# ChaissonLab/LRA

Hardware: AMD Instinct MI355X
Metric: aligned Gbp/s, 30 kb ONT vs GRCh38 (MapRead_lowacc end to end incl. SAM text), per job (higher is better)
Workload: dtype int32

## Files before the change

### lra_amd/csrc/sdp.hip

```cpp
#include "common.h"
#include <type_traits>
#include "scan.h"
#include <algorithm>
#include <cmath>
#include <cstring>
#include <cstdlib>
#include <string>
#include <vector>
#include <rocprim/rocprim.hpp>

namespace {

constexpr int LV = 18;
constexpr uint32_t NONE = 0xFFFFFFFFu;
constexpr int MAXALN = 16;

__device__ __forceinline__ void wave_sync() {
  __builtin_amdgcn_fence(__ATOMIC_RELEASE, "workgroup");
  __builtin_amdgcn_wave_barrier();
  __builtin_amdgcn_fence(__ATOMIC_ACQUIRE, "workgroup");
}
__device__ __forceinline__ int wave_incl_scan(int v, int lane) {
  (void)lane;
#define LRA_DPP_ADD(ctrl_, rmask_) v += __builtin_amdgcn_update_dpp(0, v, (ctrl_), (rmask_), 0xf, false)
  LRA_DPP_ADD(0x111, 0xf);
  LRA_DPP_ADD(0x112, 0xf);
  LRA_DPP_ADD(0x114, 0xf);
// ... 196 lines not shown
  const float rt = rate_in ? rate_in[r] : rate;
  for (uint64_t g = fragOff[r] + threadIdx.x; g < fragOff[r + 1]; g += blockDim.x) { fval[g] = flen[g] * rt; fprevNode[g] = NONE; fprevInd[g] = NONE; fflags[g] = 3; }
  if (threadIdx.x == 0) status[r] = 0;
}

struct BuildArgs {
  int r0, n;
  const uint32_t* order;
  const uint64_t* ptOff;
  const uint32_t* hq; const uint32_t* ht; const uint8_t* hfl; const uint32_t* h2; const uint64_t* key3; const uint32_t* pay3;
  uint32_t* scratch;
  uint32_t* cntEntries; uint32_t* cntNodes; uint32_t* cntD; uint32_t* cntV; uint32_t* cntRC;
  const ReadArena* ra;
  uint32_t* status;
  unsigned long long* stat;
};

template <int NW>
__device__ __forceinline__ int blk_incl_scan(int v, int lane, int wave, int* s_w, int& total) {
  const int inc = wave_incl_scan(v, lane);
  if (NW == 1) { total = __builtin_amdgcn_readlane(inc, 63); return inc; }
  if (lane == 63) s_w[wave] = inc;
  __syncthreads();
  int pre = 0, tot = 0;
#pragma unroll
  for (int w = 0; w < NW; w++) { const int x = s_w[w]; tot += x; if (w < wave) pre += x; }
  __syncthreads();
  total = tot;
  return inc + pre;
}
template <bool EMIT, int NW, int MODE = 0, int OCC = 8, bool BSTAT = false>
__global__ void __launch_bounds__(64 * NW, NW == 1 ? OCC : 1) sdp_build(BuildArgs a) {
  constexpr int NT = 64 * NW;
  constexpr bool LDSV = MODE == 1, NARROW = MODE != 0;
  using IT = typename std::conditional<NARROW, uint16_t, uint32_t>::type;
  using DT = typename std::conditional<NARROW, uint32_t, long long>::type;
  constexpr IT INONE = (IT)~(IT)0;
  extern __shared__ __attribute__((aligned(16))) char dyn_lds[];
  __shared__ int s_w[4][NW == 1 ? 1 : NW];
  __shared__ unsigned long long s_bt[BSTAT ? 8 : 1];
  unsigned long long btPrev = 0;
  constexpr bool bstat = BSTAT;
  if (bstat) { if (threadIdx.x < 8) s_bt[threadIdx.x] = 0; btPrev = __builtin_amdgcn_s_memtime(); }
#define BTICK(k_) do { if (bstat) { const unsigned long long t__ = __builtin_amdgcn_s_memtime(); if (threadIdx.x == 0) s_bt[k_] += t__ - btPrev; btPrev = t__; } } while (0)
  const int rr = (int)a.order[blockIdx.x], r = a.r0 + rr, tid = threadIdx.x, lane = tid & 63, wave = tid >> 6;
  auto SYNC = [&]() { if (NW == 1) wave_sync(); else __syncthreads(); };
  const uint64_t p0 = a.ptOff[r], pc0 = a.ptOff[a.r0];
  const int P = (int)(a.ptOff[r + 1] - p0);
  if (P == 0) { if (tid == 0) { if (!EMIT) { a.cntEntries[rr] = 0; a.cntNodes[rr] = 0; a.cntD[rr] = 0; } a.cntV[rr] = 0; a.cntRC[rr] = 0; } return; }
  const uint32_t* hq = a.hq + p0; const uint32_t* ht = a.ht + p0; const uint32_t* h2 = a.h2 + p0;
  const uint64_t* key3 = a.key3 + p0; const uint32_t* pay3 = a.pay3 + p0;
  uint32_t* S = a.scratch + 34 * (p0 - pc0) + 64 * (uint64_t)rr;
  const int NCAP = P + 2;
  uint32_t* tbl = S + 8 * P + 2;
  uint32_t* tmp = tbl + 12 * NCAP;
  IT* eb_ = LDSV ? (IT*)dyn_lds : (IT*)S;
  IT* rowOf = eb_; IT* colOf = rowOf + P;
  IT* lp = colOf + P;
  IT* ln = lp + 2 * P;
  IT* pf = ln + 2 * P;
  IT* ph = pf + P + 1;
  IT* ll = NARROW ? ph + P + 1 : (IT*)(tmp + 8 * NCAP);
  DT* ld = LDSV ? (DT*)(dyn_lds + ((((size_t)(10 * P + 2) * sizeof(IT)) + 7) & ~(size_t)7)) : NARROW ? (DT*)(tmp + 8 * NCAP) : (DT*)(ll + 2 * P);
  auto LN = [&](int idx) -> uint32_t { const IT v = ln[idx]; return v == INONE ? NONE : (uint32_t)v; };
#define TB(c, f, k) tbl[((c) * 6 + (f)) * NCAP + (k)]
#define TM(f, k) tmp[(f) * NCAP + (k)]
  enum { F_LS, F_LE, F_SB, F_SE, F_EB, F_EE };
  enum { T_C1S, T_C1E, T_ND, T_NE, T_CH0, T_CH1, T_BASE, T_GID };
  int R = 0, C = 0;
  for (int i0 = 0; i0 < P; i0 += NT) {
    const int i = i0 + tid;
    const int head = (i < P) && (i == 0 || hq[i] != hq[i - 1]);
    int tot; const int inc = blk_incl_scan<NW>(head, lane, wave, s_w[0], tot);
    if (i < P) rowOf[i] = R + inc - 1;
    R += tot;
  }
  for (int i0 = 0; i0 < P; i0 += NT) {
    const int i = i0 + tid;
    const int head = (i < P) && (i == 0 || ht[h2[i]] != ht[h2[i - 1]]);
    int tot; const int inc = blk_incl_scan<NW>(head, lane, wave, s_w[0], tot);
    if (i < P) colOf[h2[i]] = C + inc - 1;
// ... 32 lines not shown
    const bool col = fam & 1, back = fam >= 2, desc = (fam == 1 || fam == 2), swapped = (fam == 3);
    const IT* lineOf = col ? colOf : rowOf;
    const int nLines = col ? C : R;
    const int sc = back ? 2 : 0;
    const int nS = cOff[sc + 1] - cOff[sc], nEn = cOff[sc + 2] - cOff[sc + 1], Pf = nS + nEn;
    if (nS == 0 || nEn == 0) continue;
    const int fam2 = fam & 1;
    const int dSide = swapped ? 1 : 0, eSide = swapped ? 0 : 1;
    for (int i = tid; i < Pf; i += NT) {
      const uint32_t pos = pay3[cOff[sc] + i];
      lp[i] = (IT)pos; ln[i] = 0; ll[i] = lineOf[pos];
      ld[i] = (DT)(back ? (long long)ht[pos] + hq[pos] : (long long)ht[pos] - hq[pos]);
    }
    if (tid == 0) { TB(0, F_LS, 0) = 0; TB(0, F_LE, 0) = nLines; TB(0, F_SB, 0) = 0; TB(0, F_SE, 0) = nS; TB(0, F_EB, 0) = nS; TB(0, F_EE, 0) = Pf; }
    int nNodes = 1, cur = 0;
    SYNC();
    BTICK(7);
    for (int level = 0; nNodes > 0 && !outgrown; level++) {
      if (level >= LV) { overflow = true; break; }
      const int nxt = cur ^ 1;
      IT* lpc = lp + cur * P; IT* lpn = lp + nxt * P;
      IT* llc = ll + cur * P; IT* lln = ll + nxt * P;
      DT* ldc = ld + (size_t)cur * P; DT* ldn = ld + (size_t)nxt * P;
      {
        int carry = 0;
        constexpr int UA = 4;
        for (int i0 = 0; i0 < Pf; i0 += UA * NT) {
          uint32_t kk[UA]; uint32_t ss[UA], ee[UA]; IT lv[UA]; int ff[UA];
#pragma unroll
          for (int u = 0; u < UA; u++) { const int i = i0 + u * NT + tid; kk[u] = i < Pf ? LN(i) : NONE; lv[u] = i < Pf ? llc[i] : (IT)0; }
#pragma unroll
          for (int u = 0; u < UA; u++) { ss[u] = 0; ee[u] = 0; if (kk[u] != NONE) { ss[u] = TB(cur, F_LS, kk[u]); ee[u] = TB(cur, F_LE, kk[u]); } }
#pragma unroll
          for (int u = 0; u < UA; u++) ff[u] = kk[u] == NONE ? 0 : (ee[u] - ss[u] > 1) ? (lv[u] < ((ss[u] + ee[u]) >> 1)) : 1;
#pragma unroll
          for (int u = 0; u < UA; u++) {
            const int i = i0 + u * NT + tid;
            if (i0 + u * NT >= Pf) break;
            int tot; const int inc = blk_incl_scan<NW>(ff[u], lane, wave, s_w[0], tot);
            if (i < Pf) pf[i] = (IT)(carry + inc - ff[u]);
            carry += tot;
          }
        }
        if (tid == 0) pf[Pf] = (IT)carry;
      }
      SYNC();
      BTICK(1);
      for (int k = tid; k < nNodes; k += NT) {
        TM(T_C1S, k) = (uint32_t)pf[TB(cur, F_SE, k)] - (uint32_t)pf[TB(cur, F_SB, k)];
        TM(T_C1E, k) = (uint32_t)pf[TB(cur, F_EE, k)] - (uint32_t)pf[TB(cur, F_EB, k)];
      }
      SYNC();
      {
        constexpr int UC = 2;
        for (int i0 = 0; i0 < Pf; i0 += UC * NT) {
          uint32_t kk[UC], pi0[UC], pi1[UC], sb[UC], c1[UC], psb[UC]; IT vlp[UC], vll[UC]; DT vld[UC];
#pragma unroll
          for (int u = 0; u < UC; u++) {
            const int i = i0 + u * NT + tid;
            kk[u] = NONE; pi0[u] = 0; pi1[u] = 0; vlp[u] = 0; vll[u] = 0; vld[u] = 0;
            if (i < Pf) { kk[u] = LN(i); pi0[u] = (uint32_t)pf[i]; pi1[u] = (uint32_t)pf[i + 1]; vlp[u] = lpc[i]; vll[u] = llc[i]; vld[u] = ldc[i]; }
          }
#pragma unroll
          for (int u = 0; u < UC; u++) {
            const int i = i0 + u * NT + tid;
            const bool isS = i < nS;
            sb[u] = 0; c1[u] = 0;
            if (kk[u] != NONE) { sb[u] = isS ? TB(cur, F_SB, kk[u]) : TB(cur, F_EB, kk[u]); c1[u] = isS ? TM(T_C1S, kk[u]) : TM(T_C1E, kk[u]); }
          }
#pragma unroll
          for (int u = 0; u < UC; u++) psb[u] = kk[u] != NONE ? (uint32_t)pf[sb[u]] : 0;
#pragma unroll
          for (int u = 0; u < UC; u++) {
            const int i = i0 + u * NT + tid;
            if (i >= Pf) continue;
            if (kk[u] == NONE) { ln[P + i] = INONE; continue; }
            const uint32_t rank1 = pi0[u] - psb[u];
            const uint32_t first = pi1[u] - pi0[u];
            const uint32_t np_ = first ? sb[u] + rank1 : sb[u] + c1[u] + ((uint32_t)i - sb[u] - rank1);
            lpn[np_] = vlp[u]; lln[np_] = vll[u]; ldn[np_] = vld[u];
            ln[P + np_] = (IT)(2 * kk[u] + (first ? 0 : 1));
          }
        }
      }
      SYNC();
      BTICK(2);
      {
        int carry = 0;
        constexpr int UD = NW == 1 ? 4 : 2;
        for (int j0 = 0; j0 < Pf; j0 += UD * NT) {
          uint32_t k2v[UD], le[UD], ls[UD], bg[UD], c1[UD]; DT d0[UD], d1[UD]; int hd[UD];
#pragma unroll
          for (int u = 0; u < UD; u++) {
            const int j = j0 + u * NT + tid;
            k2v[u] = NONE; d0[u] = 0; d1[u] = 0;
            if (j < Pf) { k2v[u] = LN(P + j); d0[u] = ldn[j]; d1[u] = j > 0 ? ldn[j - 1] : ldn[j]; }
          }
#pragma unroll
          for (int u = 0; u < UD; u++) {
            const int j = j0 + u * NT + tid;
            const bool isS = j < nS;
            le[u] = 0; ls[u] = 0; bg[u] = 0; c1[u] = 0;
            if (k2v[u] != NONE) {
              const uint32_t k = k2v[u] >> 1;
              le[u] = TB(cur, F_LE, k); ls[u] = TB(cur, F_LS, k); bg[u] = isS ? TB(cur, F_SB, k) : TB(cur, F_EB, k); c1[u] = isS ? TM(T_C1S, k) : TM(T_C1E, k);
            }
          }
#pragma unroll
          for (int u = 0; u < UD; u++) {
            const int j = j0 + u * NT + tid;
            hd[u] = 0;
            if (k2v[u] != NONE) {
              const uint32_t side = k2v[u] & 1;
              const bool isS = j < nS;
              const bool leaf = le[u] - ls[u] == 1;
              const bool in = leaf || (int)side == (isS ? eSide : dSide);
              if (in) {
                uint32_t beg = bg[u];
                if (!leaf && side == 1) beg += c1[u];
                hd[u] = ((uint32_t)j == beg) ? 1 : (d0[u] != d1[u]);
// ... 1 lines not shown
            }
          }
#pragma unroll
          for (int u = 0; u < UD; u++) {
            const int j = j0 + u * NT + tid;
            if (j0 + u * NT >= Pf) break;
            int tot; const int inc = blk_incl_scan<NW>(hd[u], lane, wave, s_w[0], tot);
            if (j < Pf) ph[j] = (IT)(carry + inc - hd[u]);
            carry += tot;
          }
        }
        if (tid == 0) ph[Pf] = (IT)carry;
      }
      SYNC();
      BTICK(3);
      int nNext = 0;
      for (int k0 = 0; k0 < nNodes; k0 += NT) {
        const int k = k0 + tid;
        uint32_t nD = 0, nE = 0, act0 = 0, act1 = 0, full = 0;
        uint32_t ls = 0, le = 0, sb = 0, se = 0, eb = 0, ee = 0, c1S = 0, c1E = 0;
        bool leaf = false;
        if (k < nNodes) {
          ls = TB(cur, F_LS, k); le = TB(cur, F_LE, k); sb = TB(cur, F_SB, k); se = TB(cur, F_SE, k); eb = TB(cur, F_EB, k); ee = TB(cur, F_EE, k);
          c1S = TM(T_C1S, k); c1E = TM(T_C1E, k);
          leaf = le - ls == 1;
          uint32_t dB, dE, eB, eE;
          if (leaf) { dB = eb; dE = ee; eB = sb; eE = se; }
          else {
            dB = dSide == 0 ? eb : eb + c1E; dE = dSide == 0 ? eb + c1E : ee;
            eB = eSide == 0 ? sb : sb + c1S; eE = eSide == 0 ? sb + c1S : se;
          }
          nD = (uint32_t)ph[dE] - (uint32_t)ph[dB]; nE = (uint32_t)ph[eE] - (uint32_t)ph[eB];
          full = nD > 0 && nE > 0;
          if (!leaf) {
            const bool goD = nD > 0, goE = nE > 0;
            if (dSide == 0) { act0 = goD; act1 = goE; } else { act1 = goD; act0 = goE; }
          }
        }
        int totF, totEnt, totD, totC;
        const int incF = blk_incl_scan<NW>((int)full, lane, wave, s_w[0], totF), incEnt = blk_incl_scan<NW>((int)(full ? nD + nE : 0), lane, wave, s_w[1], totEnt),
                  incD = blk_incl_scan<NW>((int)(full ? nD : 0), lane, wave, s_w[2], totD), incC = blk_incl_scan<NW>((int)(act0 + act1), lane, wave, s_w[3], totC);
        if (EMIT && ((uint64_t)nNodesTot + totF > capN || (uint64_t)nEntries + totEnt > capE || (uint64_t)sumD + totD > capD)) { outgrown = true; break; }
        if (k < nNodes) {
          const uint32_t gid = nNodesTot + incF - full, base = nEntries + incEnt - (full ? nD + nE : 0), dpre = sumD + incD - (full ? nD : 0);
          TM(T_ND, k) = nD; TM(T_NE, k) = nE; TM(T_GID, k) = full ? gid : NONE; TM(T_BASE, k) = base;
          uint32_t ci = nNext + incC - (act0 + act1);
          const uint32_t med = (ls + le) >> 1;
          TM(T_CH0, k) = NONE; TM(T_CH1, k) = NONE;
          if (act0) { TM(T_CH0, k) = ci; TB(nxt, F_LS, ci) = ls; TB(nxt, F_LE, ci) = med; TB(nxt, F_SB, ci) = sb; TB(nxt, F_SE, ci) = sb + c1S;
                      TB(nxt, F_EB, ci) = eb; TB(nxt, F_EE, ci) = eb + c1E; ci++; }
          if (act1) { TM(T_CH1, k) = ci; TB(nxt, F_LS, ci) = med; TB(nxt, F_LE, ci) = le; TB(nxt, F_SB, ci) = sb + c1S; TB(nxt, F_SE, ci) = se;
                      TB(nxt, F_EB, ci) = eb + c1E; TB(nxt, F_EE, ci) = ee; }
          if (EMIT && full) {
            Node nd;
            nd.dBase = base; nd.nD = nD; nd.nE = nE; nd.last = -1; nd.sTop = 1; nd.nBlk = 0;
            nd.stkOff = 2 * dpre + 4 * gid; nd.blkOff = blkPair + 2 * base + 8 * gid; nd.stkCap = 2 * nD + 4; nd.blkCap = 2 * (nD + nE) + 8;
            nd.eLast = 0;
            nodesR[gid] = nd;
            stkR[nd.stkOff] = make_int2(-1, (int)nE + 1);
          }
        }
        nNodesTot += totF; nEntries += totEnt; sumD += totD; nNext += totC;
      }
      if (outgrown) break;
      SYNC();
      BTICK(4);
      {
        constexpr int UF = 2;
        for (int j0 = 0; j0 < Pf; j0 += UF * NT) {
          uint32_t k2v[UF], le[UF], ls[UF], ch[UF], gidv[UF], bg[UF], c1[UF], nNE[UF], nND[UF], bs[UF], p0v[UF], p1v[UF], pbg[UF], posv[UF], tq[UF], tt[UF];
#pragma unroll
          for (int u = 0; u < UF; u++) {
            const int j = j0 + u * NT + tid;
            k2v[u] = NONE; p0v[u] = 0; p1v[u] = 0; posv[u] = 0;
            if (j < Pf) { k2v[u] = LN(P + j); if (EMIT) { p0v[u] = (uint32_t)ph[j]; p1v[u] = (uint32_t)ph[j + 1]; posv[u] = lpn[j]; } }
          }
#pragma unroll
          for (int u = 0; u < UF; u++) {
            const int j = j0 + u * NT + tid;
            const bool isS = j < nS;
            le[u] = 0; ls[u] = 0; ch[u] = 0; gidv[u] = NONE; bg[u] = 0; c1[u] = 0; nNE[u] = 0; nND[u] = 0; bs[u] = 0; tq[u] = 0; tt[u] = 0;
            if (k2v[u] != NONE) {
              const uint32_t k = k2v[u] >> 1, side = k2v[u] & 1;
              le[u] = TB(cur, F_LE, k); ls[u] = TB(cur, F_LS, k); ch[u] = side == 0 ? TM(T_CH0, k) : TM(T_CH1, k); gidv[u] = TM(T_GID, k);
              if (EMIT) {
                bg[u] = isS ? TB(cur, F_SB, k) : TB(cur, F_EB, k); c1[u] = isS ? TM(T_C1S, k) : TM(T_C1E, k);
                nNE[u] = TM(T_NE, k); nND[u] = TM(T_ND, k); bs[u] = TM(T_BASE, k);
                tq[u] = hq[posv[u]]; tt[u] = ht[posv[u]];
              }
            }
          }
#pragma unroll
          for (int u = 0; u < UF; u++) {
            pbg[u] = 0;
            if (EMIT && k2v[u] != NONE) {
              const uint32_t side = k2v[u] & 1;
              const bool leaf = le[u] - ls[u] == 1;
              uint32_t beg = bg[u];
              if (!leaf && side == 1) beg += c1[u];
              bg[u] = beg;
              pbg[u] = (uint32_t)ph[beg];
// ... 21 lines not shown
                const uint32_t pos = posv[u];
                if (head) {
                  const long long dgv = back ? (long long)tt[u] + tq[u] : (long long)tt[u] - tq[u];
                  entR[ent].val = dgv;
                  if (isS && idx == n - 1) nodesR[gid].eLast = dgv;
                }
                visR[(uint64_t)pos * (2 * LV) + fam2 * LV + level] = make_uint2(gid, idx);
              }
            }
          }
        }
      }
      SYNC();
      BTICK(5);
      if (EMIT) {
        constexpr int UG = 2;
        for (int j0 = 0; j0 < Pf; j0 += UG * NT) {
          uint32_t k2v[UG], gidv[UG], le[UG], ls[UG], bg[UG], c1[UG], nDv[UG], nEv[UG], bs[UG], p0v[UG], p1v[UG], pbg[UG];
          bool on[UG];
#pragma unroll
          for (int u = 0; u < UG; u++) {
            const int j = j0 + u * NT + tid;
            k2v[u] = NONE; p0v[u] = 0; p1v[u] = 0;
            if (j < Pf) { k2v[u] = LN(P + j); p0v[u] = (uint32_t)ph[j]; p1v[u] = (uint32_t)ph[j + 1]; }
          }
#pragma unroll
          for (int u = 0; u < UG; u++) {
            const int j = j0 + u * NT + tid;
            const bool isS = j < nS;
            gidv[u] = NONE; le[u] = 0; ls[u] = 0; bg[u] = 0; c1[u] = 0; nDv[u] = 0; nEv[u] = 0; bs[u] = 0;
            if (k2v[u] != NONE && p1v[u] != p0v[u]) {
              const uint32_t k = k2v[u] >> 1;
              gidv[u] = TM(T_GID, k); le[u] = TB(cur, F_LE, k); ls[u] = TB(cur, F_LS, k);
              bg[u] = isS ? TB(cur, F_SB, k) : TB(cur, F_EB, k); c1[u] = isS ? TM(T_C1S, k) : TM(T_C1E, k);
              nDv[u] = TM(T_ND, k); nEv[u] = TM(T_NE, k); bs[u] = TM(T_BASE, k);
            }
          }
#pragma unroll
          for (int u = 0; u < UG; u++) {
            const int j = j0 + u * NT + tid;
            const bool isS = j < nS;
            const uint32_t side = k2v[u] & 1;
            const bool leaf = le[u] - ls[u] == 1;
            on[u] = k2v[u] != NONE && p1v[u] != p0v[u] && gidv[u] != NONE && (leaf || (int)side == (isS ? eSide : dSide));
            pbg[u] = 0;
            if (on[u]) { uint32_t beg = bg[u]; if (!leaf && side == 1) beg += c1[u]; pbg[u] = (uint32_t)ph[beg]; }
          }
          uint32_t entv[UG], mv[UG], lo[UG], cnt[UG]; long long xv[UG]; const Ent* opp[UG];
#pragma unroll
// ... 36 lines not shown
                if (cnt[u] > 0) { const uint32_t s2 = cnt[u] >> 1; if (go(vL[u])) { lo[u] += s2 + 1; cnt[u] -= s2 + 1; } else cnt[u] = s2; }
              }
            }
          }
#pragma unroll
          for (int u = 0; u < UG; u++) {
            if (!on[u]) continue;
            const bool isS = j0 + u * NT + tid < nS;
            const uint32_t ent = entv[u], m = mv[u];
            entR[ent].b = isS ? (int32_t)lo[u] - 1 : (lo[u] == m ? -1 : (int32_t)lo[u]);
            if (!isS) edR[ent] = lo[u] == m ? 0 : opp[u][lo[u]].val;
            entR[ent].v = 0.f; apR[ent] = 0;
          }
        }
      }
      nNodes = nNext; cur = nxt;
      SYNC();
      BTICK(6);
    }
  }
  if (bstat && tid == 0) { for (int k = 0; k < 8; k++) atomicAdd(a.stat + k, s_bt[k]); atomicAdd(a.stat + 8, (unsigned long long)P); }
  for (int o = 32; o > 0; o >>= 1) nVisits += __shfl_xor(nVisits, o);
  if (NW > 1) {
    if (lane == 0) s_w[0][wave] = (int)nVisits;
    __syncthreads();
    nVisits = 0;
    for (int w = 0; w < NW; w++) nVisits += (uint32_t)s_w[0][w];
  }
  if (tid == 0) {
    if (!EMIT) { a.cntEntries[rr] = nEntries; a.cntNodes[rr] = nNodesTot; a.cntD[rr] = sumD; a.cntV[rr] = nVisits; a.cntRC[rr] = (uint32_t)max(R, C); }
    else { a.cntV[rr] = nEntries; a.cntRC[rr] = (uint32_t)max(R, C); }
    if (overflow) atomicOr(&a.status[r], (uint32_t)LRA_ST_RANGE);
    if (outgrown) atomicOr(&a.status[r], (uint32_t)LRA_ST_CAPACITY);
  }
#undef TB
#undef TM
#undef BTICK
}

struct ProcArgs {
  int r0, n;
  const uint32_t* order;
  const uint64_t* ptOff; const uint64_t* fragOff;
  const uint8_t* hfl; const uint32_t* hfr;
  const int32_t* flen; float* fval; uint32_t* fprevNode; uint32_t* fprevInd; uint8_t* fflags;
  const float* rate_in; float rate;
  const ReadArena* ra; uint32_t* poolUsed;
  uint32_t* status;
  PwlTab pwl;
  const short* penTab; int penN;
// ... 1056 lines not shown
    a.cq[k] = a.fq[f0 + lf]; a.ct[k] = a.ft[f0 + lf]; a.clen[k] = a.flen[f0 + lf]; a.cstrand[k] = a.fstrand[f0 + lf];
    a.can[k] = a.fai[f0 + lf]; a.ccl[k] = a.fcl[f0 + lf];
  }
  a.nChains[r] = (uint32_t)nCh;
}

inline size_t sz(size_t n, size_t elem) { return (n * elem + 255) / 256 * 256; }

static long sdp_big_points(const lra_ctx* ctx, int mode) {
  if (const char* e = getenv("LRA_SDP_BIG_POINTS")) return atol(e);
  if (ctx->sdp_inner) return 1500;
  if (mode == 0) { if (const char* e = getenv("LRA_SDP_BIG_POINTS_A")) return atol(e); return 2500; }
  if (const char* e = getenv("LRA_SDP_BIG_POINTS_2")) return atol(e);
  return ctx->pipelined ? 14000 : 6000;
}
template <bool EMIT>
static void launch_small_builds(lra_ctx* ctx, const BuildArgs& ba, const uint32_t* d_order, const std::vector<uint32_t>& h_order, const uint64_t* h_pt, int from, int to) {
  static const bool noLds = getenv("LRA_SDP_BUILD_NOLDS") != nullptr;
  hipStream_t st = ctx->stream;
  auto pts = [&](int i) { return (long)(h_pt[h_order[i] + 1] - h_pt[h_order[i]]); };
  int at = from;
  const long caps[3] = {512, 256, 128};
  int cut[4];
  for (int c = 0; c < 3; c++) { while (at < to && (noLds || pts(at) > caps[c])) at++; cut[c] = at; }
  cut[3] = to;
  if (cut[0] > from) {
    int mid = from;
    while (mid < cut[0] && pts(mid) >= 16384) mid++;
    if (mid > from) { BuildArgs bb = ba; bb.order = d_order + from; hipLaunchKernelGGL((sdp_build<EMIT, 1, 0>), dim3(mid - from), dim3(64), 0, st, bb); }
    if (cut[0] > mid) {
      BuildArgs bb = ba; bb.order = d_order + mid;
      static const int occEnv = getenv("LRA_SDP_BUILD_OCC") ? atoi(getenv("LRA_SDP_BUILD_OCC")) : 0;
      const int occ = occEnv ? occEnv : ctx->pipelined ? 6 : 8;
      if (bb.stat) { if (occ == 6) hipLaunchKernelGGL((sdp_build<EMIT, 1, 2, 6, true>), dim3(cut[0] - mid), dim3(64), 0, st, bb); else hipLaunchKernelGGL((sdp_build<EMIT, 1, 2, 8, true>), dim3(cut[0] - mid), dim3(64), 0, st, bb); }
      else if (occ == 4) hipLaunchKernelGGL((sdp_build<EMIT, 1, 2, 4>), dim3(cut[0] - mid), dim3(64), 0, st, bb);
      else if (occ == 5) hipLaunchKernelGGL((sdp_build<EMIT, 1, 2, 5>), dim3(cut[0] - mid), dim3(64), 0, st, bb);
      else if (occ == 6) hipLaunchKernelGGL((sdp_build<EMIT, 1, 2, 6>), dim3(cut[0] - mid), dim3(64), 0, st, bb);
      else hipLaunchKernelGGL((sdp_build<EMIT, 1, 2>), dim3(cut[0] - mid), dim3(64), 0, st, bb);
    }
  }
  for (int c = 0; c < 3; c++) {
    const int n = cut[c + 1] - cut[c];
    if (n <= 0) continue;
    BuildArgs bb = ba; bb.order = d_order + cut[c];
    hipLaunchKernelGGL((sdp_build<EMIT, 1, 1>), dim3(n), dim3(64), (size_t)(28 * caps[c] + 32), st, bb);
  }
}

int sdp_run(lra_ctx* ctx, int n_reads, const uint64_t* d_cluster_off, const uint64_t* d_c_start, const uint32_t* d_c_count,
            const int32_t* d_c_strand, const uint32_t* d_q, const uint32_t* d_t, const int32_t* d_len, const uint64_t* d_read_off,
            const float* d_rate, const lra_sdp_opts* opts, lra_chain_result* out, const uint32_t* d_qe, const uint32_t* d_te,
            const int32_t* d_num_anchors) {
  const bool boxes = d_qe != nullptr;
// ... 184 lines not shown
        for (int i = 0; i < nr; i++) h_order[i] = (uint32_t)i;
        std::sort(h_order.begin(), h_order.end(), [&](uint32_t x, uint32_t y) {
          const uint64_t px = h_pt[r0 + x + 1] - h_pt[r0 + x], py = h_pt[r0 + y + 1] - h_pt[r0 + y];
          return px != py ? px > py : x < y;
        });
      }
      LRA_HIP_CHECK(ctx, hipMemcpyAsync(order, h_order.data(), (size_t)nr * 4, hipMemcpyHostToDevice, st));
      LRA_HIP_CHECK(ctx, hipStreamSynchronize(st));
      h_orderAll = h_order;
    }
    uint64_t* entOff = (uint64_t*)take(ws, nr1 + 1, 8); uint64_t* bytes = (uint64_t*)take(ws, nr1 + 1, 8); uint64_t* byteOff = (uint64_t*)take(ws, nr1 + 1, 8);
    ReadArena* ra = (ReadArena*)take(ws, nr1, sizeof(ReadArena));
    BuildArgs ba;
    memset(&ba, 0, sizeof ba);
    ba.r0 = r0; ba.n = nr; ba.ptOff = ptOff; ba.hq = hq; ba.ht = ht; ba.hfl = hfl; ba.h2 = pay2; ba.key3 = key1; ba.pay3 = pay1; ba.scratch = scratch;
    ba.cntEntries = cntE; ba.cntNodes = cntN; ba.cntD = cntD; ba.cntV = cntV; ba.cntRC = cntRC; ba.status = status; ba.order = order; ba.stat = nullptr;
    static const bool buildStat = getenv("LRA_SDP_BUILD_STAT") != nullptr;
    if (buildStat) { (void)hipMalloc((void**)&ba.stat, 16 * 8); (void)hipMemsetAsync(ba.stat, 0, 16 * 8, st); }
    const bool onePassEnv = !(getenv("LRA_SDP_ONEPASS") && getenv("LRA_SDP_ONEPASS")[0] == '0');
    const bool onePass = onePassEnv && !getenv("LRA_SDP_RATIOS");
    auto count_pass = [&](const uint32_t* d_ord, const std::vector<uint32_t>& h_ord, int n) {
      lra_time_begin(ctx, ctx->sdp_inner ? "sdp_inner_build_count" : "sdp_build_count");
      const long big_pts = sdp_big_points(ctx, opts->mode);
      int nb0 = 0;
      while (nb0 < n && (long)(h_pt[r0 + h_ord[nb0] + 1] - h_pt[r0 + h_ord[nb0]]) >= big_pts) nb0++;
      const bool forked = nb0 > 0 && n > nb0;
      BuildArgs bc = ba; bc.order = d_ord; bc.n = n;
      if (nb0 > 0) hipLaunchKernelGGL((sdp_build<false, 16>), dim3(nb0), dim3(1024), 0, forked ? lra_side_fork(ctx) : st, bc);
      if (n > nb0) launch_small_builds<false>(ctx, bc, d_ord, h_ord, h_pt.data() + r0, nb0, n);
      if (forked) lra_side_join(ctx);
      lra_time_end(ctx);
// ... 164 lines not shown
      h_sub.clear();
      for (int i = 0; i < nsub; i++) { const uint32_t rr = att == 0 ? h_orderAll[i] : h_prev[i]; if (h_status[rr] & LRA_ST_CAPACITY) h_sub.push_back(rr); }
      nsub = (int)h_sub.size();
      if (nsub == 0) break;
      h_prev = h_sub;
      LRA_HIP_CHECK(ctx, hipMemcpyAsync(order2, h_sub.data(), (size_t)nsub * 4, hipMemcpyHostToDevice, st));
      LRA_HIP_CHECK(ctx, hipStreamSynchronize(st));
      subOrder = order2;
    }
    if (ba.stat) {
      unsigned long long hb[16];
      (void)hipStreamSynchronize(st); (void)hipMemcpy(hb, ba.stat, sizeof hb, hipMemcpyDeviceToHost); (void)hipFree(ba.stat); ba.stat = nullptr;
      const double pts = (double)std::max<unsigned long long>(hb[8], 1);
      fprintf(stderr, "[sdp-build-stat] mode %d inner %d reads %d; the wave-per-read builds of 513 .. 16383 points, %llu points; cycles per point: set-up %.1f family %.1f | per level pass A %.1f C %.1f D %.1f E %.1f F %.1f G %.1f\n", opts->mode, (int)ctx->sdp_inner, nr,
              hb[8], hb[0] / pts, hb[7] / pts, hb[1] / pts, hb[2] / pts, hb[3] / pts, hb[4] / pts, hb[5] / pts, hb[6] / pts);
    }
    if (onePass) { int rc = read_rc(); if (rc) return rc; }
    totalEntries += totE;
    const uint64_t cf0 = h_frag[r0], cfn = h_frag[r1] - h_frag[r0];
    if (cfn > 0) {
      lra_time_begin(ctx, ctx->sdp_inner ? "sdp_inner_trace" : "sdp_trace");
      const bool needOrder = opts->mode != LRA_SDP_SINGLE_CLUSTER;
      if (needOrder) hipLaunchKernelGGL(k_valkeys, dim3((unsigned)((cfn + 255) / 256)), dim3(256), 0, st, cf0, cfn, fval, fragRead, fragOff, okey, opay);
      hipLaunchKernelGGL(k_pred, dim3((unsigned)((cfn + 255) / 256)), dim3(256), 0, st, cf0, cfn, r0, (const uint32_t*)fragRead, (const uint32_t*)fprevNode,
                         (const uint32_t*)fprevInd, (const uint32_t*)status, (const ReadArena*)ra, spare);
      lra_time_end(ctx);
      if (needOrder) { int rc = lra_sort_minimizers_batch(ctx, nr, fragOff + r0, okey, opay); if (rc) return rc; }
      TraceArgs ta;
      ta.r0 = r0; ta.n = nr; ta.numAln = opts->NumAln; ta.single = opts->mode == LRA_SDP_SINGLE_CLUSTER; ta.alnthres = opts->alnthres; ta.fragOff = fragOff; ta.read_off = d_read_off; ta.fq = fq; ta.ft = ft;
      ta.flen = flen; ta.fcl = fcl; ta.fai = fai; ta.fval = fval; ta.fpred = spare; ta.fflags = fflags; ta.opay = opay; ta.used = used;
// ... 36 lines not shown
```

Measured before the change: 1.199.

## Finish small SDP build subtrees in LDS once children fit a local cap

The level loop of the sparse DP build kernel becomes a lambda. In MODE 2 it now tracks the largest child node size. Once every child holds at most 62 points, the remaining levels run group by group in LDS: nodes are packed into groups of up to 62 points, their element arrays and node tables are copied from the global arena into LDS, and all deeper levels finish there with unroll factor 1. This aims to cut global-memory traffic for the deep levels of mid-sized reads. In exchange it adds dynamic LDS per block, which may lower occupancy, plus group partitioning and copy overhead; an env var can turn it off.

```diff
diff --git a/lra_amd/csrc/sdp.hip b/lra_amd/csrc/sdp.hip
--- a/lra_amd/csrc/sdp.hip
+++ b/lra_amd/csrc/sdp.hip
@@ -11,6 +11,7 @@
 
 namespace {
 
+constexpr int SUB_CAP = 62;
 constexpr int LV = 18;
 constexpr uint32_t NONE = 0xFFFFFFFFu;
 constexpr int MAXALN = 16;
@@ -237,6 +238,7 @@
   const ReadArena* ra;
   uint32_t* status;
   unsigned long long* stat;
+  int subCap;
 };
 
 template <int NW>
@@ -262,9 +264,10 @@
   extern __shared__ __attribute__((aligned(16))) char dyn_lds[];
   __shared__ int s_w[4][NW == 1 ? 1 : NW];
   __shared__ unsigned long long s_bt[BSTAT ? 8 : 1];
+  __shared__ unsigned long long s_bx[BSTAT ? 5 : 1];
   unsigned long long btPrev = 0;
   constexpr bool bstat = BSTAT;
-  if (bstat) { if (threadIdx.x < 8) s_bt[threadIdx.x] = 0; btPrev = __builtin_amdgcn_s_memtime(); }
+  if (bstat) { if (threadIdx.x < 8) s_bt[threadIdx.x] = 0; if (threadIdx.x < 5) s_bx[threadIdx.x] = 0; btPrev = __builtin_amdgcn_s_memtime(); }
 #define BTICK(k_) do { if (bstat) { const unsigned long long t__ = __builtin_amdgcn_s_memtime(); if (threadIdx.x == 0) s_bt[k_] += t__ - btPrev; btPrev = t__; } } while (0)
   const int rr = (int)a.order[blockIdx.x], r = a.r0 + rr, tid = threadIdx.x, lane = tid & 63, wave = tid >> 6;
   auto SYNC = [&]() { if (NW == 1) wave_sync(); else __syncthreads(); };
@@ -285,9 +288,10 @@
   IT* ph = pf + P + 1;
   IT* ll = NARROW ? ph + P + 1 : (IT*)(tmp + 8 * NCAP);
   DT* ld = LDSV ? (DT*)(dyn_lds + ((((size_t)(10 * P + 2) * sizeof(IT)) + 7) & ~(size_t)7)) : NARROW ? (DT*)(tmp + 8 * NCAP) : (DT*)(ll + 2 * P);
-  auto LN = [&](int idx) -> uint32_t { const IT v = ln[idx]; return v == INONE ? NONE : (uint32_t)v; };
 #define TB(c, f, k) tbl[((c) * 6 + (f)) * NCAP + (k)]
-#define TM(f, k) tmp[(f) * NCAP + (k)]
+#define TBC(f, k) tbC[(f) * NC + (k)]
+#define TBN(f, k) tbN[(f) * NC + (k)]
+#define TM(f, k) tm[(f) * NC + (k)]
   enum { F_LS, F_LE, F_SB, F_SE, F_EB, F_EE };
   enum { T_C1S, T_C1E, T_ND, T_NE, T_CH0, T_CH1, T_BASE, T_GID };
   int R = 0, C = 0;
@@ -350,23 +354,22 @@
     }
     if (tid == 0) { TB(0, F_LS, 0) = 0; TB(0, F_LE, 0) = nLines; TB(0, F_SB, 0) = 0; TB(0, F_SE, 0) = nS; TB(0, F_EB, 0) = nS; TB(0, F_EE, 0) = Pf; }
     int nNodes = 1, cur = 0;
+    int maxCh = Pf;
     SYNC();
     BTICK(7);
-    for (int level = 0; nNodes > 0 && !outgrown; level++) {
-      if (level >= LV) { overflow = true; break; }
-      const int nxt = cur ^ 1;
-      IT* lpc = lp + cur * P; IT* lpn = lp + nxt * P;
-      IT* llc = ll + cur * P; IT* lln = ll + nxt * P;
-      DT* ldc = ld + (size_t)cur * P; DT* ldn = ld + (size_t)nxt * P;
+    auto runLevel = [&](auto inLds, const int level, const int Pf, const int nS, const int PS, auto* lpc, auto* lpn, auto* llc, auto* lln, auto* ldc, auto* ldn,
+                        auto* ln, auto* pf, auto* ph, uint32_t* tbC, uint32_t* tbN, uint32_t* tm, const int NC, const int nNodes, int& maxCh) -> int {
+      constexpr bool L = decltype(inLds)::value;
+      auto LN = [&](int idx) -> uint32_t { const IT v = ln[idx]; return v == INONE ? NONE : (uint32_t)v; };
       {
         int carry = 0;
-        constexpr int UA = 4;
+        constexpr int UA = L ? 1 : 4;
         for (int i0 = 0; i0 < Pf; i0 += UA * NT) {
           uint32_t kk[UA]; uint32_t ss[UA], ee[UA]; IT lv[UA]; int ff[UA];
 #pragma unroll
           for (int u = 0; u < UA; u++) { const int i = i0 + u * NT + tid; kk[u] = i < Pf ? LN(i) : NONE; lv[u] = i < Pf ? llc[i] : (IT)0; }
 #pragma unroll
-          for (int u = 0; u < UA; u++) { ss[u] = 0; ee[u] = 0; if (kk[u] != NONE) { ss[u] = TB(cur, F_LS, kk[u]); ee[u] = TB(cur, F_LE, kk[u]); } }
+          for (int u = 0; u < UA; u++) { ss[u] = 0; ee[u] = 0; if (kk[u] != NONE) { ss[u] = TBC(F_LS, kk[u]); ee[u] = TBC(F_LE, kk[u]); } }
 #pragma unroll
           for (int u = 0; u < UA; u++) ff[u] = kk[u] == NONE ? 0 : (ee[u] - ss[u] > 1) ? (lv[u] < ((ss[u] + ee[u]) >> 1)) : 1;
 #pragma unroll
@@ -383,12 +386,12 @@
       SYNC();
       BTICK(1);
       for (int k = tid; k < nNodes; k += NT) {
-        TM(T_C1S, k) = (uint32_t)pf[TB(cur, F_SE, k)] - (uint32_t)pf[TB(cur, F_SB, k)];
-        TM(T_C1E, k) = (uint32_t)pf[TB(cur, F_EE, k)] - (uint32_t)pf[TB(cur, F_EB, k)];
+        TM(T_C1S, k) = (uint32_t)pf[TBC(F_SE, k)] - (uint32_t)pf[TBC(F_SB, k)];
+        TM(T_C1E, k) = (uint32_t)pf[TBC(F_EE, k)] - (uint32_t)pf[TBC(F_EB, k)];
       }
       SYNC();
       {
-        constexpr int UC = 2;
+        constexpr int UC = L ? 1 : 2;
         for (int i0 = 0; i0 < Pf; i0 += UC * NT) {
           uint32_t kk[UC], pi0[UC], pi1[UC], sb[UC], c1[UC], psb[UC]; IT vlp[UC], vll[UC]; DT vld[UC];
 #pragma unroll
@@ -402,7 +405,7 @@
             const int i = i0 + u * NT + tid;
             const bool isS = i < nS;
             sb[u] = 0; c1[u] = 0;
-            if (kk[u] != NONE) { sb[u] = isS ? TB(cur, F_SB, kk[u]) : TB(cur, F_EB, kk[u]); c1[u] = isS ? TM(T_C1S, kk[u]) : TM(T_C1E, kk[u]); }
+            if (kk[u] != NONE) { sb[u] = isS ? TBC(F_SB, kk[u]) : TBC(F_EB, kk[u]); c1[u] = isS ? TM(T_C1S, kk[u]) : TM(T_C1E, kk[u]); }
           }
 #pragma unroll
           for (int u = 0; u < UC; u++) psb[u] = kk[u] != NONE ? (uint32_t)pf[sb[u]] : 0;
@@ -410,12 +413,12 @@
           for (int u = 0; u < UC; u++) {
             const int i = i0 + u * NT + tid;
             if (i >= Pf) continue;
-            if (kk[u] == NONE) { ln[P + i] = INONE; continue; }
+            if (kk[u] == NONE) { ln[PS + i] = INONE; continue; }
             const uint32_t rank1 = pi0[u] - psb[u];
             const uint32_t first = pi1[u] - pi0[u];
             const uint32_t np_ = first ? sb[u] + rank1 : sb[u] + c1[u] + ((uint32_t)i - sb[u] - rank1);
             lpn[np_] = vlp[u]; lln[np_] = vll[u]; ldn[np_] = vld[u];
-            ln[P + np_] = (IT)(2 * kk[u] + (first ? 0 : 1));
+            ln[PS + np_] = (IT)(2 * kk[u] + (first ? 0 : 1));
           }
         }
       }
@@ -423,14 +426,14 @@
       BTICK(2);
       {
         int carry = 0;
-        constexpr int UD = NW == 1 ? 4 : 2;
+        constexpr int UD = L ? 1 : NW == 1 ? 4 : 2;
         for (int j0 = 0; j0 < Pf; j0 += UD * NT) {
           uint32_t k2v[UD], le[UD], ls[UD], bg[UD], c1[UD]; DT d0[UD], d1[UD]; int hd[UD];
 #pragma unroll
           for (int u = 0; u < UD; u++) {
             const int j = j0 + u * NT + tid;
             k2v[u] = NONE; d0[u] = 0; d1[u] = 0;
-            if (j < Pf) { k2v[u] = LN(P + j); d0[u] = ldn[j]; d1[u] = j > 0 ? ldn[j - 1] : ldn[j]; }
+            if (j < Pf) { k2v[u] = LN(PS + j); d0[u] = ldn[j]; d1[u] = j > 0 ? ldn[j - 1] : ldn[j]; }
           }
 #pragma unroll
           for (int u = 0; u < UD; u++) {
@@ -439,7 +442,7 @@
             le[u] = 0; ls[u] = 0; bg[u] = 0; c1[u] = 0;
             if (k2v[u] != NONE) {
               const uint32_t k = k2v[u] >> 1;
-              le[u] = TB(cur, F_LE, k); ls[u] = TB(cur, F_LS, k); bg[u] = isS ? TB(cur, F_SB, k) : TB(cur, F_EB, k); c1[u] = isS ? TM(T_C1S, k) : TM(T_C1E, k);
+              le[u] = TBC(F_LE, k); ls[u] = TBC(F_LS, k); bg[u] = isS ? TBC(F_SB, k) : TBC(F_EB, k); c1[u] = isS ? TM(T_C1S, k) : TM(T_C1E, k);
             }
           }
 #pragma unroll
@@ -471,14 +474,14 @@
       }
       SYNC();
       BTICK(3);
-      int nNext = 0;
+      int nNext = 0, mc = 0;
       for (int k0 = 0; k0 < nNodes; k0 += NT) {
         const int k = k0 + tid;
         uint32_t nD = 0, nE = 0, act0 = 0, act1 = 0, full = 0;
         uint32_t ls = 0, le = 0, sb = 0, se = 0, eb = 0, ee = 0, c1S = 0, c1E = 0;
         bool leaf = false;
         if (k < nNodes) {
-          ls = TB(cur, F_LS, k); le = TB(cur, F_LE, k); sb = TB(cur, F_SB, k); se = TB(cur, F_SE, k); eb = TB(cur, F_EB, k); ee = TB(cur, F_EE, k);
+          ls = TBC(F_LS, k); le = TBC(F_LE, k); sb = TBC(F_SB, k); se = TBC(F_SE, k); eb = TBC(F_EB, k); ee = TBC(F_EE, k);
           c1S = TM(T_C1S, k); c1E = TM(T_C1E, k);
           leaf = le - ls == 1;
           uint32_t dB, dE, eB, eE;
@@ -504,10 +507,11 @@
           uint32_t ci = nNext + incC - (act0 + act1);
           const uint32_t med = (ls + le) >> 1;
           TM(T_CH0, k) = NONE; TM(T_CH1, k) = NONE;
-          if (act0) { TM(T_CH0, k) = ci; TB(nxt, F_LS, ci) = ls; TB(nxt, F_LE, ci) = med; TB(nxt, F_SB, ci) = sb; TB(nxt, F_SE, ci) = sb + c1S;
-                      TB(nxt, F_EB, ci) = eb; TB(nxt, F_EE, ci) = eb + c1E; ci++; }
-          if (act1) { TM(T_CH1, k) = ci; TB(nxt, F_LS, ci) = med; TB(nxt, F_LE, ci) = le; TB(nxt, F_SB, ci) = sb + c1S; TB(nxt, F_SE, ci) = se;
-                      TB(nxt, F_EB, ci) = eb + c1E; TB(nxt, F_EE, ci) = ee; }
+          if (act0) { TM(T_CH0, k) = ci; TBN(F_LS, ci) = ls; TBN(F_LE, ci) = med; TBN(F_SB, ci) = sb; TBN(F_SE, ci) = sb + c1S;
+                      TBN(F_EB, ci) = eb; TBN(F_EE, ci) = eb + c1E; ci++; }
+          if (act1) { TM(T_CH1, k) = ci; TBN(F_LS, ci) = med; TBN(F_LE, ci) = le; TBN(F_SB, ci) = sb + c1S; TBN(F_SE, ci) = se;
+                      TBN(F_EB, ci) = eb + c1E; TBN(F_EE, ci) = ee; }
+          if (MODE == 2) { if (act0) mc = max(mc, (int)(c1S + c1E)); if (act1) mc = max(mc, (int)(se - sb - c1S + ee - eb - c1E)); }
           if (EMIT && full) {
             Node nd;
             nd.dBase = base; nd.nD = nD; nd.nE = nE; nd.last = -1; nd.sTop = 1; nd.nBlk = 0;
@@ -519,18 +523,19 @@
         }
         nNodesTot += totF; nEntries += totEnt; sumD += totD; nNext += totC;
       }
-      if (outgrown) break;
+      if (outgrown) return 0;
+      if (MODE == 2) { for (int o = 32; o > 0; o >>= 1) mc = max(mc, __shfl_xor(mc, o)); maxCh = __builtin_amdgcn_readfirstlane(mc); }
       SYNC();
       BTICK(4);
       {
-        constexpr int UF = 2;
+        constexpr int UF = L ? 1 : 2;
         for (int j0 = 0; j0 < Pf; j0 += UF * NT) {
           uint32_t k2v[UF], le[UF], ls[UF], ch[UF], gidv[UF], bg[UF], c1[UF], nNE[UF], nND[UF], bs[UF], p0v[UF], p1v[UF], pbg[UF], posv[UF], tq[UF], tt[UF];
 #pragma unroll
           for (int u = 0; u < UF; u++) {
             const int j = j0 + u * NT + tid;
             k2v[u] = NONE; p0v[u] = 0; p1v[u] = 0; posv[u] = 0;
-            if (j < Pf) { k2v[u] = LN(P + j); if (EMIT) { p0v[u] = (uint32_t)ph[j]; p1v[u] = (uint32_t)ph[j + 1]; posv[u] = lpn[j]; } }
+            if (j < Pf) { k2v[u] = LN(PS + j); if (EMIT) { p0v[u] = (uint32_t)ph[j]; p1v[u] = (uint32_t)ph[j + 1]; posv[u] = lpn[j]; } }
           }
 #pragma unroll
           for (int u = 0; u < UF; u++) {
@@ -539,9 +544,9 @@
             le[u] = 0; ls[u] = 0; ch[u] = 0; gidv[u] = NONE; bg[u] = 0; c1[u] = 0; nNE[u] = 0; nND[u] = 0; bs[u] = 0; tq[u] = 0; tt[u] = 0;
             if (k2v[u] != NONE) {
               const uint32_t k = k2v[u] >> 1, side = k2v[u] & 1;
-              le[u] = TB(cur, F_LE, k); ls[u] = TB(cur, F_LS, k); ch[u] = side == 0 ? TM(T_CH0, k) : TM(T_CH1, k); gidv[u] = TM(T_GID, k);
+              le[u] = TBC(F_LE, k); ls[u] = TBC(F_LS, k); ch[u] = side == 0 ? TM(T_CH0, k) : TM(T_CH1, k); gidv[u] = TM(T_GID, k);
               if (EMIT) {
-                bg[u] = isS ? TB(cur, F_SB, k) : TB(cur, F_EB, k); c1[u] = isS ? TM(T_C1S, k) : TM(T_C1E, k);
+                bg[u] = isS ? TBC(F_SB, k) : TBC(F_EB, k); c1[u] = isS ? TM(T_C1S, k) : TM(T_C1E, k);
                 nNE[u] = TM(T_NE, k); nND[u] = TM(T_ND, k); bs[u] = TM(T_BASE, k);
                 tq[u] = hq[posv[u]]; tt[u] = ht[posv[u]];
               }
@@ -593,7 +598,7 @@
       SYNC();
       BTICK(5);
       if (EMIT) {
-        constexpr int UG = 2;
+        constexpr int UG = L ? 1 : 2;
         for (int j0 = 0; j0 < Pf; j0 += UG * NT) {
           uint32_t k2v[UG], gidv[UG], le[UG], ls[UG], bg[UG], c1[UG], nDv[UG], nEv[UG], bs[UG], p0v[UG], p1v[UG], pbg[UG];
           bool on[UG];
@@ -601,7 +606,7 @@
           for (int u = 0; u < UG; u++) {
             const int j = j0 + u * NT + tid;
             k2v[u] = NONE; p0v[u] = 0; p1v[u] = 0;
-            if (j < Pf) { k2v[u] = LN(P + j); p0v[u] = (uint32_t)ph[j]; p1v[u] = (uint32_t)ph[j + 1]; }
+            if (j < Pf) { k2v[u] = LN(PS + j); p0v[u] = (uint32_t)ph[j]; p1v[u] = (uint32_t)ph[j + 1]; }
           }
 #pragma unroll
           for (int u = 0; u < UG; u++) {
@@ -610,8 +615,8 @@
             gidv[u] = NONE; le[u] = 0; ls[u] = 0; bg[u] = 0; c1[u] = 0; nDv[u] = 0; nEv[u] = 0; bs[u] = 0;
             if (k2v[u] != NONE && p1v[u] != p0v[u]) {
               const uint32_t k = k2v[u] >> 1;
-              gidv[u] = TM(T_GID, k); le[u] = TB(cur, F_LE, k); ls[u] = TB(cur, F_LS, k);
-              bg[u] = isS ? TB(cur, F_SB, k) : TB(cur, F_EB, k); c1[u] = isS ? TM(T_C1S, k) : TM(T_C1E, k);
+              gidv[u] = TM(T_GID, k); le[u] = TBC(F_LE, k); ls[u] = TBC(F_LS, k);
+              bg[u] = isS ? TBC(F_SB, k) : TBC(F_EB, k); c1[u] = isS ? TM(T_C1S, k) : TM(T_C1E, k);
               nDv[u] = TM(T_ND, k); nEv[u] = TM(T_NE, k); bs[u] = TM(T_BASE, k);
             }
           }
@@ -678,12 +683,69 @@
           }
         }
       }
-      nNodes = nNext; cur = nxt;
       SYNC();
       BTICK(6);
-    }
-  }
-  if (bstat && tid == 0) { for (int k = 0; k < 8; k++) atomicAdd(a.stat + k, s_bt[k]); atomicAdd(a.stat + 8, (unsigned long long)P); }
+      return nNext;
+    };
+    for (int level = 0; nNodes > 0 && !outgrown; level++) {
+      if (level >= LV) { overflow = true; break; }
+      if constexpr (MODE == 2) {
+        if (a.subCap > 0 && maxCh <= SUB_CAP) {
+          constexpr int CS = SUB_CAP, NC2 = CS;
+          IT* lpL = (IT*)dyn_lds; IT* llL = lpL + 2 * CS; IT* lnL = llL + 2 * CS; IT* pfL = lnL + 2 * CS; IT* phL = pfL + CS + 1;
+          DT* ldL = (DT*)(dyn_lds + (((size_t)(8 * CS + 2) * sizeof(IT) + 7) & ~(size_t)7));
+          const uint32_t* tbL = tbl + cur * 6 * NCAP;
+          uint32_t* tA = (uint32_t*)(ldL + 2 * CS); uint32_t* tB = tA + 6 * NC2; uint32_t* tmL = tB + 6 * NC2;
+          if (bstat && tid == 0) { s_bx[2]++; s_bx[3] += (unsigned long long)level; }
+          int maxLv = level;
+          for (int k0 = 0; k0 < nNodes && !outgrown && !overflow;) {
+            const uint32_t s0 = tbL[F_SB * NCAP + k0], e0 = tbL[F_EB * NCAP + k0];
+            int k1 = nNodes;
+            for (int kb = k0 + 1; kb < nNodes; kb += 64) {
+              const int k = kb + lane;
+              const bool brk = k >= nNodes || (tbL[F_SE * NCAP + k] - s0) + (tbL[F_EE * NCAP + k] - e0) > (uint32_t)CS;
+              const unsigned long long m = __ballot(brk);
+              if (m) { k1 = kb + (int)__builtin_ctzll(m); break; }
+            }
+            k1 = __builtin_amdgcn_readfirstlane(k1);
+            const uint32_t s1 = tbL[F_SE * NCAP + k1 - 1], e1 = tbL[F_EE * NCAP + k1 - 1];
+            const int nSg = (int)(s1 - s0), Pg = nSg + (int)(e1 - e0), ng = k1 - k0;
+            for (int i = lane; i < Pg; i += 64) {
+              const int src = i < nSg ? (int)s0 + i : (int)e0 + (i - nSg);
+              const IT kv = ln[src];
+              lpL[i] = lp[cur * P + src]; llL[i] = ll[cur * P + src]; ldL[i] = ld[(size_t)cur * P + src];
+              lnL[i] = kv == INONE ? INONE : (IT)(kv - k0);
+            }
+            for (int k = lane; k < ng; k += 64) {
+              tA[F_LS * NC2 + k] = tbL[F_LS * NCAP + k0 + k]; tA[F_LE * NC2 + k] = tbL[F_LE * NCAP + k0 + k];
+              tA[F_SB * NC2 + k] = tbL[F_SB * NCAP + k0 + k] - s0; tA[F_SE * NC2 + k] = tbL[F_SE * NCAP + k0 + k] - s0;
+              tA[F_EB * NC2 + k] = tbL[F_EB * NCAP + k0 + k] - e0 + nSg; tA[F_EE * NC2 + k] = tbL[F_EE * NCAP + k0 + k] - e0 + nSg;
+            }
+            SYNC();
+            int n2 = ng, c2 = 0, lv = level, mcg = 0;
+            for (; n2 > 0 && !outgrown; lv++) {
+              if (lv >= LV) { overflow = true; break; }
+              if (bstat && tid == 0) s_bx[1] += (unsigned long long)Pg;
+              n2 = runLevel(std::true_type(), lv, Pg, nSg, CS, lpL + c2 * CS, lpL + (c2 ^ 1) * CS, llL + c2 * CS, llL + (c2 ^ 1) * CS, ldL + c2 * CS, ldL + (c2 ^ 1) * CS,
+                            lnL, pfL, phL, c2 ? tB : tA, c2 ? tA : tB, tmL, NC2, n2, mcg);
+              c2 ^= 1;
+            }
+            maxLv = max(maxLv, lv);
+            k0 = k1;
+          }
+          if (bstat && tid == 0) s_bx[4] += (unsigned long long)(maxLv - level);
+          break;
+        }
+      }
+      if (bstat && tid == 0) s_bx[0] += (unsigned long long)Pf;
+      const int nxt = cur ^ 1;
+      nNodes = runLevel(std::false_type(), level, Pf, nS, P, lp + cur * P, lp + nxt * P, ll + cur * P, ll + nxt * P, ld + (size_t)cur * P, ld + (size_t)nxt * P, ln, pf, ph,
+                        tbl + cur * 6 * NCAP, tbl + nxt * 6 * NCAP, tmp, NCAP, nNodes, maxCh);
+      cur = nxt;
+    }
+  }
+  if (bstat && tid == 0) { for (int k = 0; k < 8; k++) atomicAdd(a.stat + k, s_bt[k]); atomicAdd(a.stat + 8, (unsigned long long)P);
+                           for (int k = 0; k < 5; k++) atomicAdd(a.stat + 9 + k, s_bx[k]); }
   for (int o = 32; o > 0; o >>= 1) nVisits += __shfl_xor(nVisits, o);
   if (NW > 1) {
     if (lane == 0) s_w[0][wave] = (int)nVisits;
@@ -698,6 +760,8 @@
     if (outgrown) atomicOr(&a.status[r], (uint32_t)LRA_ST_CAPACITY);
   }
 #undef TB
+#undef TBC
+#undef TBN
 #undef TM
 #undef BTICK
 }
@@ -1784,6 +1848,11 @@
   if (const char* e = getenv("LRA_SDP_BIG_POINTS_2")) return atol(e);
   return ctx->pipelined ? 14000 : 6000;
 }
+static int sdp_build_subtree_on() {
+  const char* e = getenv("LRA_SDP_BUILD_SUBTREE");
+  return !e || atoi(e) != 0;
+}
+static size_t sdp_build_subtree_lds(bool on) { return on ? (((size_t)(8 * SUB_CAP + 2) * 2 + 7) & ~(size_t)7) + (size_t)8 * SUB_CAP + (size_t)4 * 20 * SUB_CAP : 0; }
 template <bool EMIT>
 static void launch_small_builds(lra_ctx* ctx, const BuildArgs& ba, const uint32_t* d_order, const std::vector<uint32_t>& h_order, const uint64_t* h_pt, int from, int to) {
   static const bool noLds = getenv("LRA_SDP_BUILD_NOLDS") != nullptr;
@@ -1799,14 +1868,15 @@
     while (mid < cut[0] && pts(mid) >= 16384) mid++;
     if (mid > from) { BuildArgs bb = ba; bb.order = d_order + from; hipLaunchKernelGGL((sdp_build<EMIT, 1, 0>), dim3(mid - from), dim3(64), 0, st, bb); }
     if (cut[0] > mid) {
-      BuildArgs bb = ba; bb.order = d_order + mid;
+      BuildArgs bb = ba; bb.order = d_order + mid; bb.subCap = !noLds && sdp_build_subtree_on();
+      const size_t lds = sdp_build_subtree_lds(bb.subCap);
       static const int occEnv = getenv("LRA_SDP_BUILD_OCC") ? atoi(getenv("LRA_SDP_BUILD_OCC")) : 0;
       const int occ = occEnv ? occEnv : ctx->pipelined ? 6 : 8;
-      if (bb.stat) { if (occ == 6) hipLaunchKernelGGL((sdp_build<EMIT, 1, 2, 6, true>), dim3(cut[0] - mid), dim3(64), 0, st, bb); else hipLaunchKernelGGL((sdp_build<EMIT, 1, 2, 8, true>), dim3(cut[0] - mid), dim3(64), 0, st, bb); }
-      else if (occ == 4) hipLaunchKernelGGL((sdp_build<EMIT, 1, 2, 4>), dim3(cut[0] - mid), dim3(64), 0, st, bb);
-      else if (occ == 5) hipLaunchKernelGGL((sdp_build<EMIT, 1, 2, 5>), dim3(cut[0] - mid), dim3(64), 0, st, bb);
-      else if (occ == 6) hipLaunchKernelGGL((sdp_build<EMIT, 1, 2, 6>), dim3(cut[0] - mid), dim3(64), 0, st, bb);
-      else hipLaunchKernelGGL((sdp_build<EMIT, 1, 2>), dim3(cut[0] - mid), dim3(64), 0, st, bb);
+      if (bb.stat) { if (occ == 6) hipLaunchKernelGGL((sdp_build<EMIT, 1, 2, 6, true>), dim3(cut[0] - mid), dim3(64), lds, st, bb); else hipLaunchKernelGGL((sdp_build<EMIT, 1, 2, 8, true>), dim3(cut[0] - mid), dim3(64), lds, st, bb); }
+      else if (occ == 4) hipLaunchKernelGGL((sdp_build<EMIT, 1, 2, 4>), dim3(cut[0] - mid), dim3(64), lds, st, bb);
+      else if (occ == 5) hipLaunchKernelGGL((sdp_build<EMIT, 1, 2, 5>), dim3(cut[0] - mid), dim3(64), lds, st, bb);
+      else if (occ == 6) hipLaunchKernelGGL((sdp_build<EMIT, 1, 2, 6>), dim3(cut[0] - mid), dim3(64), lds, st, bb);
+      else hipLaunchKernelGGL((sdp_build<EMIT, 1, 2>), dim3(cut[0] - mid), dim3(64), lds, st, bb);
     }
   }
   for (int c = 0; c < 3; c++) {
@@ -2021,7 +2091,7 @@
     BuildArgs ba;
     memset(&ba, 0, sizeof ba);
     ba.r0 = r0; ba.n = nr; ba.ptOff = ptOff; ba.hq = hq; ba.ht = ht; ba.hfl = hfl; ba.h2 = pay2; ba.key3 = key1; ba.pay3 = pay1; ba.scratch = scratch;
-    ba.cntEntries = cntE; ba.cntNodes = cntN; ba.cntD = cntD; ba.cntV = cntV; ba.cntRC = cntRC; ba.status = status; ba.order = order; ba.stat = nullptr;
+    ba.cntEntries = cntE; ba.cntNodes = cntN; ba.cntD = cntD; ba.cntV = cntV; ba.cntRC = cntRC; ba.status = status; ba.order = order; ba.stat = nullptr; ba.subCap = 0;
     static const bool buildStat = getenv("LRA_SDP_BUILD_STAT") != nullptr;
     if (buildStat) { (void)hipMalloc((void**)&ba.stat, 16 * 8); (void)hipMemsetAsync(ba.stat, 0, 16 * 8, st); }
     const bool onePassEnv = !(getenv("LRA_SDP_ONEPASS") && getenv("LRA_SDP_ONEPASS")[0] == '0');
@@ -2216,6 +2286,9 @@
       const double pts = (double)std::max<unsigned long long>(hb[8], 1);
       fprintf(stderr, "[sdp-build-stat] mode %d inner %d reads %d; the wave-per-read builds of 513 .. 16383 points, %llu points; cycles per point: set-up %.1f family %.1f | per level pass A %.1f C %.1f D %.1f E %.1f F %.1f G %.1f\n", opts->mode, (int)ctx->sdp_inner, nr,
               hb[8], hb[0] / pts, hb[7] / pts, hb[1] / pts, hb[2] / pts, hb[3] / pts, hb[4] / pts, hb[5] / pts, hb[6] / pts);
+      const double el = (double)std::max<unsigned long long>(hb[9] + hb[10], 1), fams = (double)std::max<unsigned long long>(hb[11], 1);
+      fprintf(stderr, "[sdp-build-stat] (element, level) pairs: %llu from the arena, %llu in LDS (%.1f %%); %llu families reach phase 2, at level %.2f on average, %.2f levels there\n",
+              hb[9], hb[10], 100.0 * hb[10] / el, hb[11], hb[12] / fams, hb[13] / fams);
     }
     if (onePass) { int rc = read_rc(); if (rc) return rc; }
     totalEntries += totE;
```

Measured after the change: 1.217, median of 6. +1.5%, better.
